# luanaruiz9/gated_gcrnns

Measured on AMD Instinct MI355X. Metric: sequences/sec (node), N=1000 K=5 T=32 F=64, higher is better.
Workload: dtype bf16

## Files before the change

### gated_gcrnns_amd/_lib.py

```python
import ctypes as C
import os

import torch

from . import build as _build

F32, F64, BF16 = 0, 1, 2

_c_i64 = C.c_int64
_c_p = C.c_void_p


class GcrnnError(RuntimeError):
    pass


def _load():
    path = os.environ.get('GCRNN_LIBPATH')
    if path:
        return _bind(C.CDLL(path))
    path = _build.LIBPATH
    if _build.needs_build() and os.path.exists(_build.HIPCC):
        _build.build(verbose=False)
    if not os.path.exists(path):
# ... 38 lines not shown
        'gcrnn_taps_backward_weight_parts': (C.c_int, [_c_i64, _c_i64, _c_i64, _c_i64, C.POINTER(_c_i64), C.POINTER(_c_i64)]),
        'gcrnn_taps_backward_weight': (C.c_int, [C.c_int, _c_p, _c_p, _c_p, _c_i64, _c_p, _c_p, C.c_double,
                                                 _c_i64, _c_i64, _c_i64, _c_i64, _c_p]),
        'gcrnn_ell_size': (C.c_int, [_c_p, _c_i64, _c_p, C.c_int, C.c_int, _c_i64, C.POINTER(_c_i64)]),
        'gcrnn_ell_fill': (C.c_int, [_c_p, _c_p, _c_p, _c_i64, _c_p, C.c_int, C.c_int, _c_i64, _c_p, _c_p, _c_p, _c_p]),
        'gcrnn_ell_assign_rows_z': (C.c_int, [_c_p, _c_p, _c_i64, _c_p, C.c_int, _c_i64, _c_i64, _c_p]),
        'gcrnn_ell_fill_z': (C.c_int, [_c_p, _c_p, _c_p, _c_i64, _c_p, C.c_int, C.c_int, _c_i64, _c_p, _c_i64, _c_p, _c_p, _c_p]),
        'gcrnn_ell_assign_rows': (C.c_int, [_c_p, _c_p, _c_i64, _c_p, C.c_int, _c_i64, _c_p]),
        'gcrnn_fused_supported': (C.c_int, [_c_i64, _c_i64, _c_i64, _c_i64]),
        'gcrnn_fused_padded_nodes': (_c_i64, []),
        'gcrnn_fused_step_waves': (_c_i64, []),
        'gcrnn_fused_wgrad_waves': (_c_i64, []),
        'gcrnn_pack_seq_major': (C.c_int, [C.c_int, _c_p, _c_p, _c_i64, _c_i64, _c_i64, _c_i64, _c_i64, _c_p, _c_p]),
        'gcrnn_pack_seq_major_padded': (C.c_int, [_c_p, _c_p] + [_c_i64] * 6 + [_c_p]),
        'gcrnn_unpack_seq_major': (C.c_int, [C.c_int, _c_p, _c_p, _c_i64, _c_i64, _c_i64, _c_i64, _c_i64, _c_p, _c_p]),
        'gcrnn_fused_pack_weights': (C.c_int, [C.c_int, _c_p, _c_p, _c_p, _c_i64, _c_i64, _c_i64, _c_i64, _c_p]),
        'gcrnn_fused_forward_bf16': (C.c_int, [_c_p, _c_p, _c_p, _c_p, _c_p, _c_p, _c_p, _c_p, _c_p, _c_p, _c_p,
                                               _c_p, _c_p,
                                               _c_i64, _c_i64, _c_i64, _c_i64, _c_i64, _c_i64, _c_i64, _c_p, C.c_int, _c_p, C.c_double, _c_p, _c_p, _c_p, _c_p]),
        'gcrnn_fused_pack_weights_wide': (C.c_int, [C.c_int, _c_p, _c_p, _c_p, _c_i64, _c_i64, _c_i64, _c_i64, _c_i64, C.c_double, _c_p]),
        'gcrnn_fused_forward_wide_supported': (C.c_int, [_c_i64] * 7 + [C.c_double, C.c_int, C.c_int]),
        'gcrnn_fused_forward_wide_bf16': (C.c_int, [_c_p] * 10 + [_c_i64] * 7 + [_c_p, C.c_int, _c_p, _c_p, _c_p, _c_p]),
        'gcrnn_fused_forward_wide_scratch_bytes': (_c_i64, [_c_i64, _c_i64, C.c_int]),
        'gcrnn_fused_forward_wide_scratch_bf16': (C.c_int, [_c_p] * 3 + [_c_i64] + [_c_p] * 7 + [_c_i64] * 7 + [_c_p, C.c_int, _c_p, _c_p, _c_p, _c_p]),
        'gcrnn_fused_backward_data_wide_supported': (C.c_int, [_c_i64] * 6 + [C.c_double, C.c_int, C.c_int]),
        'gcrnn_fused_backward_data_wide_bf16': (C.c_int, [_c_p] * 8 + [_c_i64] * 6 + [_c_p] * 7),
        'gcrnn_gate_readout_finish': (C.c_int, [_c_p, _c_i64, _c_p, _c_p, _c_p, _c_p, _c_i64, _c_p]),
        'gcrnn_fused_filter_output_wide_supported': (C.c_int, [_c_i64] * 7 + [C.c_double, C.c_int, C.c_int]),
        'gcrnn_fused_filter_output_wide_bf16': (C.c_int, [_c_p] * 7 + [_c_i64] * 7 + [_c_p, _c_p]),
        'gcrnn_fused_node_forward_wide_supported': (C.c_int, [_c_i64] * 6 + [C.c_double, C.c_int]),
        'gcrnn_fused_node_forward_wide_bf16': (C.c_int, [_c_p] * 11 + [_c_i64] * 6 + [_c_p, C.c_int, _c_p]),
        'gcrnn_fused_gate_pair_wide_supported': (C.c_int, [_c_i64] * 7 + [C.c_double, C.c_int, C.c_int]),
        'gcrnn_fused_gate_pair_prepass_wide_bf16': (C.c_int, [_c_p] * 12 + [_c_i64] * 7 + [_c_p, _c_p, _c_p, _c_p]),
        'gcrnn_fused_gate_pair_prepass_taps_wide_bf16': (C.c_int, [_c_p] * 7 + [_c_i64] + [_c_p] * 5 + [_c_i64] * 7 + [_c_p, _c_p, _c_p, _c_p]),
        'gcrnn_fused_inline_pack_supported': (C.c_int, [_c_i64, _c_i64, _c_i64, _c_i64, _c_i64, C.c_double]),
        'gcrnn_fused_seq_steps_per_launch': (_c_i64, [_c_i64] * 7 + [C.c_double, C.c_int, C.c_int, C.c_int]),
        'gcrnn_fused_filter_output_bf16': (C.c_int, [_c_p] * 11 + [_c_i64] * 7 + [C.c_double, C.c_int, _c_p]),
        'gcrnn_fused_node_forward_bf16': (C.c_int, [_c_p] * 15 + [_c_i64] * 6 + [_c_p, C.c_int, C.c_double, _c_p]),
        'gcrnn_fused_node_backward_data_bf16': (C.c_int, [_c_p] * 12 + [_c_i64] * 6 + [C.c_double, _c_p, C.c_int, _c_p]),
        'gcrnn_node_cell_backward': (C.c_int, [_c_p] * 11 + [_c_i64] * 5 + [_c_p]),
        'gcrnn_node_gate_dot': (C.c_int, [_c_p, _c_p, _c_p, _c_i64, _c_i64, _c_i64, _c_i64, _c_i64, _c_p]),
        'gcrnn_node_gate_dot_backward': (C.c_int, [_c_p, _c_p, _c_p, _c_p, _c_i64, _c_i64, _c_i64, _c_i64, _c_i64, _c_p]),
        'gcrnn_fused_edge_attention_supported': (C.c_int, [_c_i64, _c_i64]),
        'gcrnn_fused_edge_attention_bf16': (C.c_int, [_c_p] * 13 + [_c_i64] * 5 + [C.c_double, _c_p]),
        'gcrnn_fused_edge_attention_backward_supported': (C.c_int, [_c_i64, _c_i64, _c_i64]),
        'gcrnn_fused_edge_attention_backward_bf16': (C.c_int, [_c_p] * 14 + [_c_i64] * 6 + [C.c_double, _c_p]),
# ... 96 lines not shown
```

### gated_gcrnns_amd/csrc/gcrnn_fused_seq32.h

```cpp
#pragma once

#if defined(GCRNN_SEQ_STAMPS)
static __device__ unsigned long long gcrnn_seq32_stamps[256 * 96];
static __device__ __forceinline__ void gcrnn_stamp32_put(uint32_t lds_addr) {
  const unsigned long long tv = __builtin_amdgcn_s_memtime();
  asm volatile("ds_write_b64 %0, %1" ::"v"(lds_addr), "v"(tv) : "memory");
}
static __device__ __forceinline__ unsigned long long gcrnn_stamp32_get(uint32_t lds_addr) {
  unsigned long long tv;
  asm volatile("ds_read_b64 %0, %1\n\ts_waitcnt lgkmcnt(0)" : "=v"(tv) : "v"(lds_addr) : "memory");
  return tv;
}
#define GCRNN_STAMP32(slot)                                                                                   \
  do {                                                                                                        \
    if (wave == 0 && stamp_on && lane_now() == 0) gcrnn_stamp32_put((uint32_t)reinterpret_cast<uintptr_t>(smem) + M::FLAG_OFF + 8 * (slot)); \
  } while (0)
#define GCRNN_STAMP32_WAVE(slot0)                                                                             \
  do {                                                                                                        \
    if (stamp_on && lane_now() == 0) gcrnn_stamp32_put((uint32_t)reinterpret_cast<uintptr_t>(smem) + M::FLAG_OFF + 8 * ((slot0) + wave)); \
  } while (0)
#define GCRNN_STAMP32_FLUSH()                                                                                 \
  do {                                                                                                        \
    __syncthreads();                                                                                          \
    if (threadIdx.x < 96 && blockIdx.x < 256) gcrnn_seq32_stamps[blockIdx.x * 96 + threadIdx.x] = gcrnn_stamp32_get((uint32_t)reinterpret_cast<uintptr_t>(smem) + M::FLAG_OFF + 8 * threadIdx.x); \
// ... 56 lines not shown
  const int32_t* tile_nodes; const int32_t* tile_off; const uint2* ell_col4;
  int entries, B, N;
  const uint16_t* pk_src0; int64_t pksrc_stride;
  uint16_t* pk_dst0; int64_t pkdst_stride;
  int pk_stride;
  int nsteps;
  const float* gi0; const float* gf0; int64_t gstride;
  int hmod;
  const int32_t* flags;
  const float* gw;
  const uint4* tapf; float* taps_out; int ntaps;
  float* go;
  uint16_t* out1;
  const uint16_t* dh0_; int64_t dhstride;
  const uint16_t* hs0; int64_t hsstride;
  const float* gsc0; int64_t gscstride;
  float* gpart0; int64_t gpartstride;
  int final_raw;
  uint16_t* final_out; const uint16_t* final_h;
  const float* ng0; int64_t ngstride; int64_t nghalf;
  const float* r1a; const float* r1b;
  int stagger;
  uint16_t* scr;
};

__device__ __forceinline__ int lane_now() {
  int ln;
  asm volatile("v_mbcnt_lo_u32_b32 %0, -1, 0\n\tv_mbcnt_hi_u32_b32 %0, -1, %0" : "=v"(ln));
  return ln;
}

#define GCRNN_HOP_ASM_WIDE32_STREAM(D)                                                             \
  do {                                                                                             \
    const int gwbeg = tbeg[0] >> 2, gwend = tend[STILES - 1] >> 2;                                 \
    if (gwbeg < gwend) {                                                                           \
      const int ls_ = lane_now(), r = ls_ & 15, q = ls_ >> 4;                                      \
      const uint32_t colb = lds_col + r * 8 + (q >> 1) * 4;        \
      const uint32_t qh_ = (uint32_t)(q & 1) << 4;                                                 \
      asm volatile(GCRNN_HOP_ASM_WIDE32_TEXT                                                       \
                   : "+v"(D[0][0]), "+v"(D[0][1]), "+v"(D[1][0]), "+v"(D[1][1]), "+v"(D[2][0]), "+v"(D[2][1]), "+v"(D[3][0]), "+v"(D[3][1]), \
                     "+v"(D[4][0]), "+v"(D[4][1]), "+v"(D[5][0]), "+v"(D[5][1]), "+v"(D[6][0]), "+v"(D[6][1]), "+v"(D[7][0]), "+v"(D[7][1])  \
                   : "s"(GCRNN_SGPR(tend[0] >> 2)), "s"(GCRNN_SGPR(tend[1] >> 2)), "s"(GCRNN_SGPR(tend[2] >> 2)), "s"(GCRNN_SGPR(tend[3] >> 2)), \
                     "s"(GCRNN_SGPR(tend[4] >> 2)), "s"(GCRNN_SGPR(tend[5] >> 2)), "s"(GCRNN_SGPR(tend[6] >> 2)), "s"(GCRNN_SGPR(tend[7] >> 2)), \
                     "s"(GCRNN_SGPR(gwbeg)), "s"(GCRNN_SGPR(gwend - 1)), "v"(colb), "v"(qh_)               \
                   : GCRNN_HOP_ASM_WIDE32_CLOBBERS);                                               \
    }                                                                                              \
  } while (0)

template <int K, int HS, int XS>
struct Seq32Map {
  static constexpr int KS = HS + XS;
  static constexpr int PL = GCRNN_HOP_WIDE_PLANE;
  static constexpr int RS2 = 4 * NP + 16;
  static constexpr int BIAS_OFF = PL + 32 * 1024;
  static constexpr int FLAG_OFF = BIAS_OFF + 256;
  static constexpr int WOFF = 2 * PL;
  static constexpr int WB = K * KS * 2048;
  static constexpr int COL_OFF = WOFF + WB;
  static constexpr int NPCK = 128;
  static constexpr int PFS = 256;
  static_assert(16 * RS2 <= BIAS_OFF && FLAG_OFF + 768 <= WOFF, "LDS map");
  static size_t lds_bytes(int64_t entries, bool inline_pack, bool r1 = false) {
    const size_t need = (size_t)COL_OFF + (size_t)entries * 32 + GCRNN_HOP_COLUMN_PAD + NP * 4 + (r1 ? 2 * NP * 4 : 0) + (inline_pack ? (size_t)(32 * (XS > 0 ? XS : HS)) * NPCK * 2 : 0)
                        + PFS;
    return need <= 160 * 1024 ? need : 0;
  }
};

template <int K, int HS, int XS, int VAR, int MODE = 0, bool GATED = false, bool R1 = false, bool SPLIT = false>
__global__ __launch_bounds__(STHREADS) void fused_seq32_kernel(const Seq32Args a) {
  static_assert(!R1 || !SPLIT, "rank-1 graphs: every mode of the persistent form (the BPTT chain takes the adjoint plan: the factors swap)");
  static_assert(!SPLIT || ((MODE == 0 || MODE == 2) && !R1 && HS > 1), "split sequences: the (un-gated or time-gated) forward and the BPTT chain, with more than one chunk");
  constexpr bool ITEMS = (MODE == 1 || MODE == 3);
  constexpr bool SONLY = (MODE == 2 || MODE == 4);
  constexpr bool PKV = (VAR & 1) != 0, USERV = (VAR & 2) != 0 && (MODE == 0 || MODE == 4);
  constexpr bool SCRV = (VAR & 4) != 0;
  static_assert(!SCRV || (MODE == 0 && !SPLIT && (VAR & 2) != 0), "state scratch: the persistent forward with the user-layout output");
  constexpr int SCR_CH = NP * 64;
  static_assert(MODE == 0 || ((MODE >= 1 && MODE <= 4) && !GATED), "modes");
  static_assert(MODE < 3 || (!R1 && !SPLIT), "modes 3, 4: uniform-weight graphs, persistent form");
  using M = Seq32Map<K, HS, XS>;
  constexpr int KS = HS + XS;
  constexpr int F = 32 * HS, G = 32 * XS;
  constexpr int NCH = (MODE == 1) ? 2 * HS : HS;
  constexpr int PL = M::PL, WOFF = M::WOFF, WB = M::WB, COL_OFF = M::COL_OFF, RS2 = M::RS2;
  constexpr int NPCK = M::NPCK, NRND = NP / NPCK, NH = NCH * (K - 1), RPH = (NRND + NH - 1) / NH;
  constexpr int PKROWS = SONLY ? F : G;
  static_assert(STILES == 8 && GCRNN_HOP_ASM && K >= 2 && (SONLY ? XS == 0 : XS > 0), "generated hop stream: 8 tiles per wave; the chain's operand is the state alone");
  extern __shared__ __attribute__((aligned(16))) char smem[];
  const int entries = a.entries, B = a.B, N = a.N;

  const int tid = threadIdx.x, lane = tid & 63;
  const int wave = __builtin_amdgcn_readfirstlane(tid >> 6);
  const int r = lane & 15, q = lane >> 4;
  constexpr int NSPL = SPLIT ? HS : 1;
  const int wg_seq = (int)blockIdx.x / NSPL, chunk0 = SPLIT ? (int)blockIdx.x % NSPL : 0, gseq = (int)gridDim.x / NSPL;
  if (wg_seq >= B) return;

  int tbeg[STILES], tend[STILES];
#pragma unroll
// ... 41 lines not shown
          const float bv = b4[e];
          const float f = kind == 0 ? bv : (bv == 0.f ? 1.f : (kind == 1 ? __builtin_amdgcn_rcpf(bv) : bv));
          ac[h4 + e][0] *= f; ac[h4 + e][1] *= f;
        }
      }
    }
  };

  {
    const int cbytes = entries * 32;
    const char* csrc = reinterpret_cast<const char*>(a.ell_col4);
    for (int p = wave; p * 1024 < cbytes; p += SWAVES)
      if (p * 1024 + lane * 16 < cbytes)
        __builtin_amdgcn_global_load_lds((const __attribute__((address_space(1))) void*)(csrc + p * 1024 + lane * 16),
                                         (__attribute__((address_space(3))) void*)(smem + COL_OFF + p * 1024), 16, 0, 0);
    const char* wsrc = reinterpret_cast<const char*>(a.wpack) + (size_t)chunk0 * WB;
    for (int p = wave; p < WB / 1024; p += SWAVES)
      __builtin_amdgcn_global_load_lds((const __attribute__((address_space(1))) void*)(wsrc + p * 1024 + lane * 16),
                                       (__attribute__((address_space(3))) void*)(smem + WOFF + p * 1024), 16, 0, 0);
    asm volatile("s_waitcnt vmcnt(0)" ::: "memory");
  }
  if (tid < GCRNN_HOP_COLUMN_PAD / 4) reinterpret_cast<uint32_t*>(smem + COL_OFF + entries * 32)[tid] = 0u;
  float* lbias = reinterpret_cast<float*>(smem + M::BIAS_OFF);
  if (tid < NCH * 32) lbias[tid] = a.bias ? a.bias[tid] : 0.f;
  __syncthreads();

  if (a.stagger > 0) {
    const unsigned long long t0 = __builtin_amdgcn_s_memtime();
    const unsigned long long d = (unsigned long long)((blockIdx.x >> 3) & 7) * (unsigned long long)a.stagger;
    while (__builtin_amdgcn_s_memtime() - t0 < d) __builtin_amdgcn_s_sleep(16);
  }
  const uint32_t lds0 = (uint32_t)reinterpret_cast<uintptr_t>(smem);
  if (lds0 != 0) __builtin_trap();
  const uint32_t lds_col = lds0 + COL_OFF;
  char* xtile = wtab + NP * 4 + (R1 ? 2 * NP * 4 : 0);

  const int skip_hi = __builtin_amdgcn_readfirstlane((MODE == 3 || (MODE == 1 && a.flags && a.flags[0] != 0)) ? 1 : 0);
  const bool skip_h = skip_hi != 0;
  bf16x8 bfr[STILES][KS];
  auto load_first_operand = [&](int b) {
    const __amdgpu_buffer_rsrc_t rsrc_h = __builtin_amdgcn_make_buffer_rsrc(const_cast<uint16_t*>(a.hfirst), 0, skip_h ? 0 : (ITEMS ? a.hmod : B) * (NP * F * 2), 0x00020000);
    const __amdgpu_buffer_rsrc_t rsrc_x = __builtin_amdgcn_make_buffer_rsrc(const_cast<uint16_t*>(a.x0), 0, XS > 0 ? B * (NP * G * 2) : 0, 0x00020000);
    const int bh = ITEMS ? __builtin_amdgcn_readfirstlane(b % a.hmod) : b;
    const int ln0 = lane_now(), qo = ln0 >> 4;
    int sw[STILES];
    slot_words(ln0, sw);
#pragma unroll
    for (int s = 0; s < KS; ++s) {
#pragma unroll
      for (int i = 0; i < STILES; ++i) {
        const int w = sw[i];
        if (s < HS)
          bfr[i][s] = __builtin_bit_cast(bf16x8, __builtin_amdgcn_raw_buffer_load_b128(rsrc_h, (w >> 16) * (F * 2) + 16 * qo + 64 * s, bh * (NP * F * 2), 0));
        else
          bfr[i][s] = __builtin_bit_cast(bf16x8, __builtin_amdgcn_raw_buffer_load_b128(rsrc_x, (w >> 16) * (G * 2) + 16 * qo + 64 * (s - HS), b * (NP * G * 2), 0));
      }
    }
  };
  bool have_operand = false;
  for (int b = wg_seq; b < B; b += gseq) {
  if (!have_operand) load_first_operand(b);
  have_operand = false;
#pragma unroll 1
  for (int step = 0; step < a.nsteps; ++step) {
    const bool fin = (MODE == 2) && a.final_raw && step == a.nsteps - 1;
    uint16_t* hout = fin ? a.final_out : (a.out0 ? a.out0 + (int64_t)step * a.ostride : nullptr);
    [[maybe_unused]] const uint16_t* ep_dh = (SONLY && !fin && a.dh0_) ? a.dh0_ + (int64_t)step * a.dhstride : nullptr;
    [[maybe_unused]] const float* ep_ng = (MODE == 4) ? a.ng0 + (int64_t)step * a.ngstride : nullptr;
    [[maybe_unused]] const uint16_t* ep_h = (MODE == 2) ? (fin ? a.final_h : (a.hs0 ? a.hs0 + (int64_t)step * a.hsstride : nullptr)) : nullptr;
    [[maybe_unused]] float* gpart = (MODE == 2 && a.gpart0) ? a.gpart0 + (int64_t)step * a.gpartstride : nullptr;
    [[maybe_unused]] float gsc = 1.f;
    if constexpr (MODE == 2) {
      if (a.gsc0) gsc = __builtin_bit_cast(float, __builtin_amdgcn_readfirstlane(__builtin_bit_cast(int, a.gsc0[(int64_t)step * a.gscstride + b])));
    }
    float gin = 1.f, gfo = 1.f, gratio = 1.f;
    if constexpr (MODE == 4) {
      if (a.gi0) {
        gin = __builtin_bit_cast(float, __builtin_amdgcn_readfirstlane(__builtin_bit_cast(int, a.gi0[(int64_t)step * a.gstride + b])));
        gfo = __builtin_bit_cast(float, __builtin_amdgcn_readfirstlane(__builtin_bit_cast(int, a.gf0[(int64_t)step * a.gstride + b])));
      }
    }
    if constexpr (GATED) {
      gin = __builtin_bit_cast(float, __builtin_amdgcn_readfirstlane(__builtin_bit_cast(int, a.gi0[(int64_t)step * a.gstride + b])));
// ... 599 lines not shown
```

### gated_gcrnns_amd/csrc/gcrnn_fused_seq32.hip

```cpp
#include "gcrnn_fused_step.h"
#include "gcrnn_fused_seq32.h"

template <typename W>
__global__ void pack_weights_wide_kernel(const W* __restrict__ wA, const W* __restrict__ wB, uint16_t* __restrict__ out,
                                         int Fout, int F, int G, int Kin, int Kst, int K, float w) {
  const int KS = (F + G) / 32;
  const int64_t total = (int64_t)(Fout / 32) * K * 2 * KS * 64 * 8;
  const int64_t idx = (int64_t)blockIdx.x * blockDim.x + threadIdx.x;
  if (idx >= total) return;
  const int j = idx & 7, lane = (idx >> 3) & 63;
  int64_t rest = idx >> 9;
  const int s = rest % KS; rest /= KS;
  const int h = rest & 1; rest >>= 1;
  const int tap = rest % K;
  const int chunk = rest / K;
  const int m = lane & 15;
  const int f = chunk * 32 + 8 * (m >> 2) + 4 * h + (m & 3);
  const int feat = 32 * s + 8 * (lane >> 4) + j;
  float v = 0.f;
  if (feat < F) { if (tap < Kst) v = (float)wB[((int64_t)f * Kst + tap) * F + feat]; }
  else          { if (tap < Kin) v = (float)wA[((int64_t)f * Kin + tap) * G + (feat - F)]; }
  float sc = 1.f;
  for (int k = 0; k < tap; ++k) sc *= w;
  out[idx] = f2bf(v * sc);
// ... 167 lines not shown
  const size_t lds = seq32_lds<K, HS, XS>(sa.entries, inline_pack, sa.r1a != nullptr);
  if (!lds) return GCRNN_ERR_UNSUPPORTED;
  if (sa.r1a) return inline_pack ? seq32_launch_v<K, HS, XS, 1, 1, false, true>(sa, lds, st) : seq32_launch_v<K, HS, XS, 0, 1, false, true>(sa, lds, st);
  return inline_pack ? seq32_launch_v<K, HS, XS, 1, 1>(sa, lds, st) : seq32_launch_v<K, HS, XS, 0, 1>(sa, lds, st);
}

int gcrnn_seq32s_forward(const Seq32Args& sa, int K, int HS, int XS, bool inline_pack, size_t lds, hipStream_t st);

static int64_t seq32_scratch_need(int64_t B, int64_t F) {
  const int64_t wgs = B < gcrnn_persistent_grid() ? B : gcrnn_persistent_grid();
  return wgs * (F / 32 - 1) * (int64_t)NP * 64;
}

extern "C" int64_t gcrnn_fused_forward_wide_scratch_bytes(int64_t B, int64_t F, int rank1) {
  if (B <= 0 || F <= 0 || F % 32) return -1;
  const char* sw = getenv("GCRNN_SEQ32_STATE_SCRATCH");
  if (sw && sw[0] == '0') return -1;
  const char* p32 = getenv("GCRNN_SEQ32P");
  if (p32 && p32[0] != '0') return -1;
  if (!rank1 && !seq32_wanted(B) && seq32_split_wanted(B, F)) return -1;
  return seq32_scratch_need(B, F);
}

static int forward_wide_impl(const void* xs, const void* h0, void* hs, void* scratch, int64_t scratch_bytes, bool no_image, const void* wpack, const float* bias,
                             const float* gi, const float* gf, const int32_t* tile_nodes, const int32_t* tile_off, const void* ell_col4, int64_t entries,
                             int64_t B, int64_t T, int64_t N, int64_t F, int64_t G, int64_t K, void* Huser,
                             int huser_last_only, const void* Xuser_inline, const float* rank1_a, const float* rank1_b,
                             void* stream) {
  if (!xs || !h0 || (!no_image && !hs) || !wpack || !tile_nodes || !tile_off || !ell_col4) return GCRNN_ERR_NULL_POINTER;
  if (no_image && !Huser) return GCRNN_ERR_NULL_POINTER;
  if ((rank1_a == nullptr) != (rank1_b == nullptr)) return GCRNN_ERR_BAD_SHAPE;
  if ((gi == nullptr) != (gf == nullptr) || (gi && Xuser_inline)) return GCRNN_ERR_BAD_SHAPE;
  if (B <= 0 || T <= 0 || N <= 0 || N > NP || B > (1 << 24) || entries <= 0 || entries % 4) return GCRNN_ERR_BAD_SHAPE;
  if (B * (NP * (F > G ? F : G) * 2) > 2147483647LL || T * F * N > 2147483647LL) return GCRNN_ERR_BAD_SHAPE;
  if (Huser && (N % 8 != 0 || (reinterpret_cast<uintptr_t>(Huser) & 15))) return GCRNN_ERR_BAD_SHAPE;
  if (Xuser_inline && (N % 8 != 0 || (reinterpret_cast<uintptr_t>(Xuser_inline) & 15) || T * G * N > 2147483647LL)) return GCRNN_ERR_BAD_SHAPE;
  if (no_image) {
    if (F % 32 || F < 32) return GCRNN_ERR_UNSUPPORTED;
    const int64_t need = seq32_scratch_need(B, F);
    if (scratch_bytes < need || (need > 0 && (!scratch || (reinterpret_cast<uintptr_t>(scratch) & 15)))) return GCRNN_ERR_BAD_SHAPE;
  }
  const int64_t xstep = B * NP * G, hstep = B * NP * F;
  Seq32Args sa{};
  sa.x0 = (const uint16_t*)xs; sa.xstride = xstep;
  sa.hfirst = (const uint16_t*)h0;
  sa.out0 = no_image ? nullptr : (uint16_t*)hs; sa.ostride = hstep;
  sa.scr = no_image ? (uint16_t*)scratch : nullptr;
  sa.wpack = (const uint4*)wpack; sa.bias = bias;
  sa.a1 = (const uint16_t*)Huser; sa.a1stride = F * N; sa.a1_last_only = huser_last_only ? 1 : 0;
  sa.ubstride = (int)((huser_last_only ? 1 : T) * F * N);
  sa.tile_nodes = tile_nodes; sa.tile_off = tile_off; sa.ell_col4 = (const uint2*)ell_col4;
  sa.entries = (int)entries; sa.B = (int)B; sa.N = (int)N;
  sa.nsteps = (int)T;
  sa.gi0 = gi; sa.gf0 = gf; sa.gstride = B;
  sa.r1a = rank1_a; sa.r1b = rank1_b;
  {
    const char* sg = getenv("GCRNN_SEQ32_STAGGER");
    sa.stagger = sg ? atoi(sg) : 0;
  }
  const bool inline_pack = Xuser_inline != nullptr && T > 2;
  if (inline_pack) {
    sa.pk_src0 = (const uint16_t*)Xuser_inline; sa.pksrc_stride = G * N;
    sa.pk_dst0 = const_cast<uint16_t*>(sa.x0); sa.pkdst_stride = xstep;
    sa.pk_stride = (int)(T * G * N);
  }
  hipStream_t st = as_stream(stream);
  const bool split = !rank1_a && !seq32_wanted(B) && seq32_split_wanted(B, F);
  if (no_image) {
    if (split) return GCRNN_ERR_UNSUPPORTED;
#define GCRNN_SEQ32_CASE(KK, HH, XX) \
    if (K == KK && F == 32 * HH && G == 32 * XX) { \
      const size_t lds = seq32_lds<KK, HH, XX>(sa.entries, inline_pack, sa.r1a != nullptr); \
      return lds ? gcrnn_seq32s_forward(sa, KK, HH, XX, inline_pack, lds, st) : GCRNN_ERR_UNSUPPORTED; \
    }
    GCRNN_SEQ32_CASE(5, 2, 2) GCRNN_SEQ32_CASE(4, 2, 2) GCRNN_SEQ32_CASE(3, 2, 2) GCRNN_SEQ32_CASE(2, 2, 2)
    GCRNN_SEQ32_CASE(5, 2, 1) GCRNN_SEQ32_CASE(4, 2, 1) GCRNN_SEQ32_CASE(3, 2, 1) GCRNN_SEQ32_CASE(2, 2, 1)
    GCRNN_SEQ32_CASE(5, 1, 1) GCRNN_SEQ32_CASE(4, 1, 1) GCRNN_SEQ32_CASE(3, 1, 1) GCRNN_SEQ32_CASE(2, 1, 1)
#undef GCRNN_SEQ32_CASE
    return GCRNN_ERR_UNSUPPORTED;
  }
  const bool pack_split = Xuser_inline != nullptr && T > 1;
  if (split && pack_split && !inline_pack) {
    sa.pk_src0 = (const uint16_t*)Xuser_inline; sa.pksrc_stride = G * N;
    sa.pk_dst0 = const_cast<uint16_t*>(sa.x0); sa.pkdst_stride = xstep;
    sa.pk_stride = (int)(T * G * N);
  }
#define GCRNN_SEQ32_CASE(KK, HH, XX) if (K == KK && F == 32 * HH && G == 32 * XX) return seq32_launch<KK, HH, XX>(sa, split ? pack_split : inline_pack, st, split, T, N);
  GCRNN_SEQ32_CASE(5, 2, 2) GCRNN_SEQ32_CASE(4, 2, 2) GCRNN_SEQ32_CASE(3, 2, 2) GCRNN_SEQ32_CASE(2, 2, 2)
  GCRNN_SEQ32_CASE(5, 2, 1) GCRNN_SEQ32_CASE(4, 2, 1) GCRNN_SEQ32_CASE(3, 2, 1) GCRNN_SEQ32_CASE(2, 2, 1)
  GCRNN_SEQ32_CASE(5, 1, 1) GCRNN_SEQ32_CASE(4, 1, 1) GCRNN_SEQ32_CASE(3, 1, 1) GCRNN_SEQ32_CASE(2, 1, 1)
#undef GCRNN_SEQ32_CASE
  return GCRNN_ERR_UNSUPPORTED;
}

extern "C" int gcrnn_fused_forward_wide_bf16(const void* xs, const void* h0, void* hs, const void* wpack, const float* bias,
                                             const float* gi, const float* gf, const int32_t* tile_nodes, const int32_t* tile_off, const void* ell_col4, int64_t entries,
                                             int64_t B, int64_t T, int64_t N, int64_t F, int64_t G, int64_t K, void* Huser,
                                             int huser_last_only, const void* Xuser_inline, const float* rank1_a, const float* rank1_b,
                                             void* stream) {
  return forward_wide_impl(xs, h0, hs, nullptr, 0, false, wpack, bias, gi, gf, tile_nodes, tile_off, ell_col4, entries, B, T, N, F, G, K, Huser,
                           huser_last_only, Xuser_inline, rank1_a, rank1_b, stream);
}

extern "C" int gcrnn_fused_forward_wide_scratch_bf16(const void* xs, const void* h0, void* scratch, int64_t scratch_bytes, const void* wpack, const float* bias,
                                                     const float* gi, const float* gf, const int32_t* tile_nodes, const int32_t* tile_off, const void* ell_col4,
                                                     int64_t entries, int64_t B, int64_t T, int64_t N, int64_t F, int64_t G, int64_t K, void* Huser,
                                                     int huser_last_only, const void* Xuser_inline, const float* rank1_a, const float* rank1_b,
                                                     void* stream) {
  return forward_wide_impl(xs, h0, nullptr, scratch, scratch_bytes, true, wpack, bias, gi, gf, tile_nodes, tile_off, ell_col4, entries, B, T, N, F, G, K, Huser,
                           huser_last_only, Xuser_inline, rank1_a, rank1_b, stream);
}


extern "C" int gcrnn_fused_gate_pair_wide_supported(int64_t B, int64_t T, int64_t N, int64_t F, int64_t G, int64_t K, int64_t entries,
                                                    double uniform_w, int img16, int with_pack) {
  if (uniform_w == 0.0 || !img16 || N <= 0 || N > NP || B <= 0 || T <= 0 || entries <= 0 || entries % 4) return 0;
  if (with_pack && (N % 8 || T * G * N > 2147483647LL)) return 0;
  if (B * T * (NP * (F > G ? F : G) * 2) > 2147483647LL) return 0;
  if (!seq32_wanted(B * T)) return 0;
  if (!seq32_lds_for(F, G, K, entries, with_pack != 0, (img16 & 2) != 0)) return 0;
  if (!with_pack) return 1;
  const int64_t first = B * T < gcrnn_persistent_grid() ? B * T : gcrnn_persistent_grid();
  return (int)((first + B - 1) / B);
}

static int gate_pair_prepass_impl(const void* x_user, void* xs, const void* h0, const void* wpack, const float* bias2,
                                  const float* gw2, float* parts, const void* tapf, float* taps_out, int64_t ntaps, void* cs_in, void* cs_f,
                                  const int32_t* tile_nodes, const int32_t* tile_off, const void* ell_col4, int64_t entries, int64_t B, int64_t T,
                                  int64_t N, int64_t F, int64_t G, int64_t K, const int32_t* h0_zero_flag,
                                  const float* rank1_a, const float* rank1_b, void* stream) {
  if (!xs || !h0 || !wpack || !tile_nodes || !tile_off || !ell_col4) return GCRNN_ERR_NULL_POINTER;
  if (tapf ? (!taps_out || ntaps <= 0 || ntaps > 16 || (reinterpret_cast<uintptr_t>(tapf) & 15)) : (!gw2 || !parts)) return GCRNN_ERR_NULL_POINTER;
  if ((rank1_a == nullptr) != (rank1_b == nullptr)) return GCRNN_ERR_NULL_POINTER;
// ... 169 lines not shown
```

### gated_gcrnns_amd/ops.py

```python
import ctypes as C
import os

import torch

from . import _lib
from ._lib import lib, check, dtype_code, GcrnnError


def _p(t):
    return C.c_void_p(t.data_ptr()) if t is not None else None


def _stream():
    return C.c_void_p(torch.cuda.current_stream().cuda_stream)


def require_device(*tensors):
    for t in tensors:
        if t is not None and not t.is_cuda:
            raise GcrnnError('gated_gcrnns_amd has no CPU path: move the module and its inputs to a ROCm '
                             'device (model.to("cuda"), x.cuda()); got a tensor on %s' % t.device)


def _pack_raw(x, perm=None):
# ... 289 lines not shown
    wpack = torch.empty(((F // 16) * K * ((F + G) // 32) * 64 * 8,), dtype=torch.bfloat16, device=dev)
    wAc, wBc = wA.contiguous(), wB.contiguous()
    check(lib.gcrnn_fused_pack_weights(dtype_code(wA.dtype), _p(wAc), _p(wBc), _p(wpack),
                                       F, G, Kin, Kst, st), 'pack_weights')
    b32 = bias.detach().float().contiguous().view(-1) if bias is not None else None
    H = torch.empty((B, T, F, N), dtype=torch.bfloat16, device=dev) if (N % 8 == 0 and user_layout) else None
    e0, e1 = torch.cuda.Event(enable_timing=True), torch.cuda.Event(enable_timing=True)
    ok = fused_inline_pack_ok(plan, N, F, G, K)
    inline_arg = inline
    inline = (ok if inline is None else (ok and inline)) and X.data_ptr() % 16 == 0
    plan16 = fused_img16_plan(graph, False, None)
    wide = fused_wide_plan(graph, B, T, N, F, G, K, inline)
    if wide is None and plan16 is None:
        inl1 = inline_arg is not False and not os.environ.get('GCRNN_NO_INLINE_PACK') and X.data_ptr() % 16 == 0
        wide = fused_wide_plan(graph, B, T, N, F, G, K, inl1, rank1=True)
        if wide is None and inl1:
            inl1 = False
            wide = fused_wide_plan(graph, B, T, N, F, G, K, False, rank1=True)
        if wide is not None:
            inline = inl1
    if wide is not None:
        wpw = _fused_pack_weights_wide(wAc, wBc, wide['uniform_w'], st)
        scr = fused_state_scratch(wide, B, F, dev) if H is not None else None
        for rep in range(reps + warm):
            if rep == warm:
                e0.record()
            _fused_forward_wide(wide, xs, h0s, hs, wAc, wBc, b32, B, T, N, F, G, K, H, False, Xc if inline else None, st, wpw=wpw, scratch=scr)
        e1.record()
        torch.cuda.synchronize()
        per_step = 1e3 * e0.elapsed_time(e1) / (reps * T)
        return {'avg_us': per_step, 'launches': reps, 'inline_pack': bool(inline), 'steps_per_launch': T,
                'launch_avg_us': per_step * T, 'kernel': 'fused_seq32_kernel'}
    for rep in range(reps + 1):
        if rep == 1:
            torch.cuda.synchronize()
            e0.record()
        check(lib.gcrnn_fused_forward_bf16(_p(xs), _p(h0s), _p(hs), _p(wpack), _p(b32), None, None, *_fused_graph_args(plan16 or plan),
                                           B, T, N, F, G, K, _p(H) if H is not None else None, 2 if plan16 else 0, None, plan.get('uniform_w', 0.0),
                                           _p(Xc) if inline else None, None, None, st),
              'fused_forward')
    e1.record()
    torch.cuda.synchronize()
    spl = int(lib.gcrnn_fused_seq_steps_per_launch(B, T, N, F, G, K, int((plan16 or plan)['entries']), float(plan.get('uniform_w', 0.0)),
                                                   1 if plan16 else 0, 1 if inline else 0, 0))
    per_step = 1e3 * e0.elapsed_time(e1) / (reps * T)
    return {'avg_us': per_step, 'launches': reps * T // max(spl, 1), 'inline_pack': bool(inline), 'steps_per_launch': max(spl, 1),
            'launch_avg_us': per_step * max(spl, 1), 'kernel': 'fused_seq_kernel' if spl else 'fused_step_kernel'}


# ... 68 lines not shown
    Kin, Kst = wA.shape[2], wB.shape[2]
    K = max(Kin, Kst)

    def make():
        wpack = torch.empty(((Fout // 32) * K * 2 * ((F + G) // 32) * 64 * 8,), dtype=torch.bfloat16, device=wA.device)
        wAc, wBc, kin = wA.contiguous(), wB.contiguous(), Kin
        if G == 0:
            wAc, kin = wBc, Kst
        check(lib.gcrnn_fused_pack_weights_wide(dtype_code(wB.dtype), _p(wAc), _p(wBc), _p(wpack), Fout, F, G, kin, Kst, float(uniform_w), st),
              'pack_weights_wide')
        return wpack
    return _cached_pack('taps32', (wA.detach(), wB.detach()), float(uniform_w), st, make)


def fused_wide_plan(graph, B, T, N, F, G, K, inline, rank1=False, gated=False):
    plan16 = fused_img16_plan(graph, False, None)
    if plan16 is None and rank1 and not os.environ.get('GCRNN_NO_IMG16'):
        plan16 = graph.fused_plan_rank1()
    if plan16 is None or F % 32 or G % 32:
        return None
    ok = lib.gcrnn_fused_forward_wide_supported(int(B), int(T), int(N), int(F), int(G), int(K), int(plan16['entries']),
                                                float(plan16.get('uniform_w', 0.0)), (3 if plan16.get('rank1') else 1) | (4 if gated else 0), 1 if inline else 0)
    return plan16 if ok else None


def fused_state_scratch(plan16, B, F, dev):
    need = int(lib.gcrnn_fused_forward_wide_scratch_bytes(int(B), int(F), 1 if plan16.get('rank1') else 0))
    if need < 0:
        return None
    return torch.empty((need,), dtype=torch.uint8, device=dev)


def _fused_forward_wide(plan16, xs, h0s, hs, wA, wB, b32, B, T, N, F, G, K, H, last_only, Xinline, st, wpw=None, gi=None, gf=None, scratch=None):
    if wpw is None:
        wpw = _fused_pack_weights_wide(wA.detach(), wB.detach(), plan16['uniform_w'], st)
    if scratch is not None:
        assert H is not None
        check(lib.gcrnn_fused_forward_wide_scratch_bf16(_p(xs), _p(h0s), _p(scratch), int(scratch.numel()), _p(wpw), _p(b32), _p(gi), _p(gf), _p(plan16['tile_slots']),
                                                        _p(plan16['tile_off']), _p(plan16['ell_col4']), plan16['entries'], B, T, N, F, G, K,
                                                        _p(H), int(bool(last_only)), _p(Xinline) if Xinline is not None else None,
                                                        _p(plan16.get('rank1_a')), _p(plan16.get('rank1_b')), st),
              'fused_forward_wide_scratch')
        return
    check(lib.gcrnn_fused_forward_wide_bf16(_p(xs), _p(h0s), _p(hs), _p(wpw), _p(b32), _p(gi), _p(gf), _p(plan16['tile_slots']), _p(plan16['tile_off']),
                                            _p(plan16['ell_col4']), plan16['entries'], B, T, N, F, G, K,
                                            _p(H) if H is not None else None, int(bool(last_only)), _p(Xinline) if Xinline is not None else None,
# ... 212 lines not shown
                       last_only=False, head=None, native_out=False):
    require_device(X, h0, wA, wB, bias)
    if packed is None and X.shape[2] < wA.shape[3]:
        if X.shape[3] % 2 == 0 and X.dtype == torch.bfloat16:
            packed = fused_pack_inputs(X, h0, graph, channels=wA.shape[3])
        else:
            Xz = X.new_zeros((X.shape[0], X.shape[1], wA.shape[3], X.shape[3]))
            Xz[:, :, :X.shape[2]] = X
            X = Xz
    elif packed is None:
        X, wA = fused_pad_operands(X, wA.detach())
    B, T, _, N = X.shape
    G = wA.shape[3]
    F = wA.shape[0]
    K = max(wA.shape[2], wB.shape[2])
    plan = graph.fused_plan()
    st = _stream()
    dev = X.device
    X = X.contiguous()
    h0 = h0.contiguous()
    events = None
    inline = False
    lean = packed is None and head is None and not return_states and not native_out and N % 8 == 0
    if packed is not None:
        xs, hs_all = packed
    elif gates is None and gate_values is None and X.data_ptr() % 16 == 0 and (
            fused_inline_pack_ok(plan, N, F, G, K) or (head is None and not os.environ.get('GCRNN_NO_INLINE_PACK')
                                                       and fused_wide_plan(graph, B, T, N, F, G, K, True, rank1=True) is not None)):
        xs, hs_all = fused_pack_inputs(X, h0, graph, first_only=True, states=not lean)
        inline = True
    elif gates is None and fused_overlap_ok(X):
        xs, hs_all, events = fused_pack_inputs(X, h0, graph, overlap=True, states=not lean)
    elif gates is not None and gate_values is None:
        xs, hs_all = fused_pack_inputs_gated(X, h0, graph, F, K, states=not lean)
    else:
        xs, hs_all = fused_pack_inputs(X, h0, graph, states=not lean)
    h0s, hs = hs_all[:1], hs_all[1:]
    gi = gf = None
    if gate_values is not None:
        gi, gf = (g.detach().float().contiguous() for g in gate_values)
        assert tuple(gi.shape) == (T, B) and tuple(gf.shape) == (T, B)
    elif gates is not None:
        hzero = fused_h0_zero_flag(h0)
        g = {}
        gp = {}
        for name in ('in', 'forget'):
# ... 2214 lines not shown
```

### include/gcrnn.h

```cpp
#ifndef GCRNN_H
#define GCRNN_H

#include <stdint.h>

#ifdef __cplusplus
extern "C" {
#endif

enum { GCRNN_F32 = 0, GCRNN_F64 = 1, GCRNN_BF16 = 2 };

enum {
  GCRNN_OK = 0,
  GCRNN_ERR_BAD_DTYPE = 1,
  GCRNN_ERR_BAD_SHAPE = 2,
  GCRNN_ERR_NULL_POINTER = 3,
  GCRNN_ERR_UNSUPPORTED = 4,
  GCRNN_ERR_LAUNCH = 5,
  GCRNN_ERR_WORKSPACE = 6
};

int gcrnn_version(void);
const char* gcrnn_status_string(int status);
const char* gcrnn_last_hip_error(void);

// ... 160 lines not shown
                             int64_t entries, int64_t B, int64_t T, int64_t N, int64_t F, int64_t G, int64_t K,
                             void* Huser, int huser_last_only, void* const* step_events, double uniform_w,
                             const void* Xuser_inline ,
                             const float* head_w ,
                             float* head_part ,
                             void* stream);

int gcrnn_fused_pack_weights_wide(int wdtype, const void* wA, const void* wB, void* wpack, int64_t Fout, int64_t F, int64_t G, int64_t Kin,
                                  int64_t Kst, double uniform_w, void* stream);
int gcrnn_fused_forward_wide_supported(int64_t B, int64_t T, int64_t N, int64_t F, int64_t G, int64_t K, int64_t entries, double uniform_w,
                                       int img16, int inline_pack);
int gcrnn_fused_forward_wide_bf16(const void* xs, const void* h0, void* hs, const void* wpack, const float* bias, const float* gi,
                                  const float* gf, const int32_t* tile_nodes, const int32_t* tile_off, const void* ell_col4, int64_t entries,
                                  int64_t B, int64_t T, int64_t N, int64_t F, int64_t G, int64_t K, void* Huser, int huser_last_only,
                                  const void* Xuser_inline,
                                  const float* rank1_a, const float* rank1_b ,
                                  void* stream);
int64_t gcrnn_fused_forward_wide_scratch_bytes(int64_t B, int64_t F, int rank1);
int gcrnn_fused_forward_wide_scratch_bf16(const void* xs, const void* h0, void* scratch, int64_t scratch_bytes, const void* wpack,
                                          const float* bias, const float* gi, const float* gf, const int32_t* tile_nodes,
                                          const int32_t* tile_off, const void* ell_col4, int64_t entries, int64_t B, int64_t T, int64_t N,
                                          int64_t F, int64_t G, int64_t K, void* Huser, int huser_last_only, const void* Xuser_inline,
                                          const float* rank1_a, const float* rank1_b, void* stream);
int gcrnn_fused_gate_pair_wide_supported(int64_t B, int64_t T, int64_t N, int64_t F, int64_t G, int64_t K, int64_t entries, double uniform_w,
                                         int img16, int with_pack);
int gcrnn_fused_backward_data_wide_supported(int64_t B, int64_t T, int64_t N, int64_t F, int64_t K, int64_t entries, double uniform_w, int img16,
                                             int inline_pack);
int gcrnn_fused_backward_data_wide_bf16(const void* dHs, const void* hs, void* dpre, void* dh0, const void* wpackT, const int32_t* tile_nodes,
                                        const int32_t* tile_off, const void* ell_col4, int64_t entries, int64_t B, int64_t T, int64_t N,
                                        int64_t F, int64_t K, const float* gf, const void* h0s, float* dgf_parts, const void* dHuser_inline,
                                        const float* rank1_a, const float* rank1_b, void* stream);
int gcrnn_fused_filter_output_wide_supported(int64_t B, int64_t T, int64_t N, int64_t F, int64_t G, int64_t K, int64_t entries, double uniform_w,
                                             int img16, int with_pack );
int gcrnn_fused_filter_output_wide_bf16(const void* xs, const void* wpack, const float* bias, void* out, const int32_t* tile_nodes,
                                        const int32_t* tile_off, const void* ell_col4, int64_t entries, int64_t B, int64_t T, int64_t N,
                                        int64_t F, int64_t G, int64_t K,
                                        const void* x_user ,
                                        void* stream);
int gcrnn_fused_node_forward_wide_supported(int64_t B, int64_t T, int64_t N, int64_t F, int64_t K, int64_t entries, double uniform_w, int img16);
int gcrnn_fused_node_forward_wide_bf16(const void* h0s, void* hs, const void* yx, const float* ngates, const float* gi, const float* gf,
                                       const void* wpackB, const float* bias, const int32_t* tile_nodes, const int32_t* tile_off,
                                       const void* ell_col4, int64_t entries, int64_t B, int64_t T, int64_t N, int64_t F, int64_t K, void* Huser,
                                       int huser_last_only, void* stream);
int gcrnn_gate_readout_finish(const float* parts, int64_t nparts, const float* lb_in, const float* lb_f, float* gi, float* gf, int64_t items,
                              void* stream);
int gcrnn_fused_gate_pair_prepass_wide_bf16(const void* x_user, void* xs, const void* h0, const void* wpack, const float* bias2,
// ... 165 lines not shown
```

Baseline: 161,800.

## Fold h0 and first input layout packing into persistent forward kernel prologue

Adds a prologue inside the persistent seq32 forward kernel that transposes the user-layout h0 and the first one or two input steps into the padded sequence-major layout. It uses LDS-staged DMA loads, swizzled reads and buffer stores. It also lets the kernel read a bf16 bias directly. This removes the separate pack and conversion launches before the forward pass on the lean path. In exchange it adds prologue work inside each per-sequence loop and passes state through a thread-local handoff set by a new API call.

```diff
diff --git a/gated_gcrnns_amd/_lib.py b/gated_gcrnns_amd/_lib.py
--- a/gated_gcrnns_amd/_lib.py
+++ b/gated_gcrnns_amd/_lib.py
@@ -84,6 +84,8 @@
         'gcrnn_fused_forward_wide_supported': (C.c_int, [_c_i64] * 7 + [C.c_double, C.c_int, C.c_int]),
         'gcrnn_fused_forward_wide_bf16': (C.c_int, [_c_p] * 10 + [_c_i64] * 7 + [_c_p, C.c_int, _c_p, _c_p, _c_p, _c_p]),
         'gcrnn_fused_forward_wide_scratch_bytes': (_c_i64, [_c_i64, _c_i64, C.c_int]),
+        'gcrnn_fused_forward_wide_user_supported': (C.c_int, [_c_i64] * 7 + [C.c_double, C.c_int]),
+        'gcrnn_fused_forward_wide_user_next': (C.c_int, [_c_p, C.c_int]),
         'gcrnn_fused_forward_wide_scratch_bf16': (C.c_int, [_c_p] * 3 + [_c_i64] + [_c_p] * 7 + [_c_i64] * 7 + [_c_p, C.c_int, _c_p, _c_p, _c_p, _c_p]),
         'gcrnn_fused_backward_data_wide_supported': (C.c_int, [_c_i64] * 6 + [C.c_double, C.c_int, C.c_int]),
         'gcrnn_fused_backward_data_wide_bf16': (C.c_int, [_c_p] * 8 + [_c_i64] * 6 + [_c_p] * 7),
diff --git a/gated_gcrnns_amd/csrc/gcrnn_fused_seq32.h b/gated_gcrnns_amd/csrc/gcrnn_fused_seq32.h
--- a/gated_gcrnns_amd/csrc/gcrnn_fused_seq32.h
+++ b/gated_gcrnns_amd/csrc/gcrnn_fused_seq32.h
@@ -102,6 +102,8 @@
   const float* r1a; const float* r1b;
   int stagger;
   uint16_t* scr;
+  const uint16_t* pro_h0;
+  int bias_bf16;
 };
 
 __device__ __forceinline__ int lane_now() {
@@ -126,6 +128,18 @@
                    : GCRNN_HOP_ASM_WIDE32_CLOBBERS);                                               \
     }                                                                                              \
   } while (0)
+
+__device__ __forceinline__ void seq32_tile_read16(uint32_t a0, uint32_t a1, uint32_t (&h0)[8], uint32_t (&h1)[8]) {
+  asm volatile("ds_read_u16 %0, %16\n\tds_read_u16 %1, %16 offset:256\n\tds_read_u16 %2, %16 offset:512\n\tds_read_u16 %3, %16 offset:768\n\t"
+               "ds_read_u16 %4, %16 offset:1024\n\tds_read_u16 %5, %16 offset:1280\n\tds_read_u16 %6, %16 offset:1536\n\tds_read_u16 %7, %16 offset:1792\n\t"
+               "ds_read_u16 %8, %17\n\tds_read_u16 %9, %17 offset:256\n\tds_read_u16 %10, %17 offset:512\n\tds_read_u16 %11, %17 offset:768\n\t"
+               "ds_read_u16 %12, %17 offset:1024\n\tds_read_u16 %13, %17 offset:1280\n\tds_read_u16 %14, %17 offset:1536\n\tds_read_u16 %15, %17 offset:1792\n\t"
+               "s_waitcnt lgkmcnt(0)"
+               : "=&v"(h0[0]), "=&v"(h0[1]), "=&v"(h0[2]), "=&v"(h0[3]), "=&v"(h0[4]), "=&v"(h0[5]), "=&v"(h0[6]), "=&v"(h0[7]),
+                 "=&v"(h1[0]), "=&v"(h1[1]), "=&v"(h1[2]), "=&v"(h1[3]), "=&v"(h1[4]), "=&v"(h1[5]), "=&v"(h1[6]), "=&v"(h1[7])
+               : "v"(a0), "v"(a1)
+               : "memory");
+}
 
 template <int K, int HS, int XS>
 struct Seq32Map {
@@ -156,6 +170,7 @@
   constexpr bool PKV = (VAR & 1) != 0, USERV = (VAR & 2) != 0 && (MODE == 0 || MODE == 4);
   constexpr bool SCRV = (VAR & 4) != 0;
   static_assert(!SCRV || (MODE == 0 && !SPLIT && (VAR & 2) != 0), "state scratch: the persistent forward with the user-layout output");
+  constexpr bool PROV = PKV && SCRV && !GATED;
   constexpr int SCR_CH = NP * 64;
   static_assert(MODE == 0 || ((MODE >= 1 && MODE <= 4) && !GATED), "modes");
   static_assert(MODE < 3 || (!R1 && !SPLIT), "modes 3, 4: uniform-weight graphs, persistent form");
@@ -243,7 +258,7 @@
   }
   if (tid < GCRNN_HOP_COLUMN_PAD / 4) reinterpret_cast<uint32_t*>(smem + COL_OFF + entries * 32)[tid] = 0u;
   float* lbias = reinterpret_cast<float*>(smem + M::BIAS_OFF);
-  if (tid < NCH * 32) lbias[tid] = a.bias ? a.bias[tid] : 0.f;
+  if (tid < NCH * 32) lbias[tid] = !a.bias ? 0.f : (a.bias_bf16 ? bf2f(reinterpret_cast<const uint16_t*>(a.bias)[tid]) : a.bias[tid]);
   __syncthreads();
 
   if (a.stagger > 0) {
@@ -278,8 +293,85 @@
       }
     }
   };
+  [[maybe_unused]] auto pro_layout = [&](auto rowsc, const uint16_t* src, uint16_t* dst, int b, int nr) __attribute__((always_inline)) {
+    constexpr int ROWS = decltype(rowsc)::value;
+    constexpr int TB = ROWS * NPCK * 2, NB = 65536 / TB;
+    constexpr int PPR = NPCK / 8, PPT = ROWS * PPR / STHREADS;
+    constexpr int PCS = ROWS / 8, NPC = NB * PCS * NPCK / STHREADS;
+    static_assert(ROWS * PPR % STHREADS == 0 && NB * TB <= M::BIAS_OFF && NPC % 2 == 0 && (STHREADS % PCS) == 0, "prologue tiles");
+    static_assert(NPCK * 2 == 256, "row pitch of the pack tile in seq32_tile_read16");
+    typedef __attribute__((__vector_size__(4 * sizeof(unsigned int)))) unsigned int u32x4_t;
+    const __amdgpu_buffer_rsrc_t rsrc_d = __builtin_amdgcn_make_buffer_rsrc(dst, 0, B * (NP * ROWS * 2), 0x00020000);
+#pragma unroll 1
+    for (int r0 = 0; r0 < nr; r0 += NB) {
+      const int tl = wave * 64 + lane_now();
+#pragma unroll
+      for (int k = 0; k < NB; ++k) {
+        if (r0 + k < nr) {
+#pragma unroll
+          for (int i = 0; i < PPT; ++i) {
+            const int id = i * STHREADS + tl;
+            const int row = id / PPR, cs = id - row * PPR;
+            const int col = (cs - (row >> 3)) & (PPR - 1);
+            if ((r0 + k) * NPCK + col * 8 < N)
+              __builtin_amdgcn_global_load_lds((const __attribute__((address_space(1))) void*)(src + (int64_t)row * N + (r0 + k) * NPCK + col * 8),
+                                               (__attribute__((address_space(3))) void*)(smem + k * TB + (i * STHREADS + wave * 64) * 16), 16, 0, GCRNN_SEQ32_NT_DMA);
+          }
+        }
+      }
+      asm volatile("s_waitcnt vmcnt(0)" ::: "memory");
+      lds_barrier();
+      u32x4_t vv[NPC];
+#pragma unroll
+      for (int j = 0; j < NPC; j += 2) {
+        uint32_t h16[2][8], sa[2];
+#pragma unroll
+        for (int e = 0; e < 2; ++e) {
+          const int k = (j + e) / (NPC / NB), id = ((j + e) % (NPC / NB)) * STHREADS + tl;
+          const int nl = id / PCS, pc = id - nl * PCS;
+          sa[e] = (uint32_t)(k * TB + (pc * 8) * (NPCK * 2) + ((nl + 8 * pc) & (NPCK - 1)) * 2);
+        }
+        seq32_tile_read16(sa[0], sa[1], h16[0], h16[1]);
+#pragma unroll
+        for (int e = 0; e < 2; ++e) {
+          const int k = (j + e) / (NPC / NB), id = ((j + e) % (NPC / NB)) * STHREADS + tl;
+          const bool ok = (r0 + k) * NPCK + id / PCS < N;
+          uint32_t w4[4];
+#pragma unroll
+          for (int jj = 0; jj < 4; ++jj) w4[jj] = h16[e][2 * jj] | (h16[e][2 * jj + 1] << 16);
+          vv[j + e] = u32x4_t{ok ? w4[0] : 0u, ok ? w4[1] : 0u, ok ? w4[2] : 0u, ok ? w4[3] : 0u};
+        }
+      }
+      int so[NPC];
+#pragma unroll
+      for (int j = 0; j < NPC; ++j) {
+        const int k = j / (NPC / NB), id = (j % (NPC / NB)) * STHREADS + tl;
+        const int nl = id / PCS, pc = id - nl * PCS;
+        so[j] = ((r0 + k) * NPCK + nl) * (ROWS * 2) + pc * 16 + b * (NP * ROWS * 2);
+      }
+#pragma unroll
+      for (int j = 0; j < NPC; ++j) asm volatile("" : "+v"(vv[j]), "+v"(so[j]));
+#pragma unroll
+      for (int j = 0; j < NPC; ++j) {
+        const int k = j / (NPC / NB);
+        if (r0 + k < nr) __builtin_amdgcn_raw_buffer_store_b128(vv[j], rsrc_d, so[j], 0, 0);
+      }
+      asm volatile("s_nop 3" ::: "memory");
+      lds_barrier();
+    }
+  };
   bool have_operand = false;
   for (int b = wg_seq; b < B; b += gseq) {
+  if constexpr (PROV) {
+    if (a.pro_h0) {
+      pro_layout(std::integral_constant<int, F>{}, a.pro_h0 + (int64_t)b * (F * N), const_cast<uint16_t*>(a.hfirst), b, NRND);
+      pro_layout(std::integral_constant<int, G>{}, a.pk_src0 + (int64_t)b * a.pk_stride, const_cast<uint16_t*>(a.x0), b, NRND);
+      if (a.nsteps > 1)
+        pro_layout(std::integral_constant<int, G>{}, a.pk_src0 + (int64_t)b * a.pk_stride + a.pksrc_stride, const_cast<uint16_t*>(a.x0) + a.xstride, b, NRND);
+      asm volatile("s_waitcnt vmcnt(0)" ::: "memory");
+      lds_barrier();
+    }
+  }
   if (!have_operand) load_first_operand(b);
   have_operand = false;
 #pragma unroll 1
diff --git a/gated_gcrnns_amd/csrc/gcrnn_fused_seq32.hip b/gated_gcrnns_amd/csrc/gcrnn_fused_seq32.hip
--- a/gated_gcrnns_amd/csrc/gcrnn_fused_seq32.hip
+++ b/gated_gcrnns_amd/csrc/gcrnn_fused_seq32.hip
@@ -213,13 +213,22 @@
   return seq32_scratch_need(B, F);
 }
 
+extern "C" int gcrnn_fused_forward_wide_user_supported(int64_t B, int64_t T, int64_t N, int64_t F, int64_t G, int64_t K, int64_t entries,
+                                                       double uniform_w, int img16) {
+  const char* sw = getenv("GCRNN_SEQ32_PROLOGUE");
+  if (sw && sw[0] == '0') return 0;
+  if (gcrnn_fused_forward_wide_scratch_bytes(B, F, (img16 & 2) != 0) < 0) return 0;
+  return gcrnn_fused_forward_wide_supported(B, T, N, F, G, K, entries, uniform_w, img16, 1);
+}
+
 static int forward_wide_impl(const void* xs, const void* h0, void* hs, void* scratch, int64_t scratch_bytes, bool no_image, const void* wpack, const float* bias,
                              const float* gi, const float* gf, const int32_t* tile_nodes, const int32_t* tile_off, const void* ell_col4, int64_t entries,
                              int64_t B, int64_t T, int64_t N, int64_t F, int64_t G, int64_t K, void* Huser,
                              int huser_last_only, const void* Xuser_inline, const float* rank1_a, const float* rank1_b,
-                             void* stream) {
+                             void* stream, const void* h0_user = nullptr, bool bias_bf16 = false) {
   if (!xs || !h0 || (!no_image && !hs) || !wpack || !tile_nodes || !tile_off || !ell_col4) return GCRNN_ERR_NULL_POINTER;
   if (no_image && !Huser) return GCRNN_ERR_NULL_POINTER;
+  if (h0_user && (!no_image || !Xuser_inline || gi || (reinterpret_cast<uintptr_t>(h0_user) & 15))) return GCRNN_ERR_BAD_SHAPE;
   if ((rank1_a == nullptr) != (rank1_b == nullptr)) return GCRNN_ERR_BAD_SHAPE;
   if ((gi == nullptr) != (gf == nullptr) || (gi && Xuser_inline)) return GCRNN_ERR_BAD_SHAPE;
   if (B <= 0 || T <= 0 || N <= 0 || N > NP || B > (1 << 24) || entries <= 0 || entries % 4) return GCRNN_ERR_BAD_SHAPE;
@@ -237,7 +246,8 @@
   sa.hfirst = (const uint16_t*)h0;
   sa.out0 = no_image ? nullptr : (uint16_t*)hs; sa.ostride = hstep;
   sa.scr = no_image ? (uint16_t*)scratch : nullptr;
-  sa.wpack = (const uint4*)wpack; sa.bias = bias;
+  sa.wpack = (const uint4*)wpack; sa.bias = bias; sa.bias_bf16 = bias_bf16 ? 1 : 0;
+  sa.pro_h0 = (const uint16_t*)h0_user;
   sa.a1 = (const uint16_t*)Huser; sa.a1stride = F * N; sa.a1_last_only = huser_last_only ? 1 : 0;
   sa.ubstride = (int)((huser_last_only ? 1 : T) * F * N);
   sa.tile_nodes = tile_nodes; sa.tile_off = tile_off; sa.ell_col4 = (const uint2*)ell_col4;
@@ -249,7 +259,7 @@
     const char* sg = getenv("GCRNN_SEQ32_STAGGER");
     sa.stagger = sg ? atoi(sg) : 0;
   }
-  const bool inline_pack = Xuser_inline != nullptr && T > 2;
+  const bool inline_pack = Xuser_inline != nullptr && (T > 2 || h0_user);
   if (inline_pack) {
     sa.pk_src0 = (const uint16_t*)Xuser_inline; sa.pksrc_stride = G * N;
     sa.pk_dst0 = const_cast<uint16_t*>(sa.x0); sa.pkdst_stride = xstep;
@@ -293,13 +303,29 @@
                            huser_last_only, Xuser_inline, rank1_a, rank1_b, stream);
 }
 
+static thread_local const void* seq32_next_h0_user = nullptr;
+static thread_local int seq32_next_bias_dtype = GCRNN_F32;
+
+extern "C" int gcrnn_fused_forward_wide_user_next(const void* h0_user, int bias_dtype) {
+  if (!h0_user) return GCRNN_ERR_NULL_POINTER;
+  if (bias_dtype != GCRNN_F32 && bias_dtype != GCRNN_BF16) return GCRNN_ERR_BAD_DTYPE;
+  if (reinterpret_cast<uintptr_t>(h0_user) & 15) return GCRNN_ERR_BAD_SHAPE;
+  seq32_next_h0_user = h0_user;
+  seq32_next_bias_dtype = bias_dtype;
+  return GCRNN_OK;
+}
+
 extern "C" int gcrnn_fused_forward_wide_scratch_bf16(const void* xs, const void* h0, void* scratch, int64_t scratch_bytes, const void* wpack, const float* bias,
                                                      const float* gi, const float* gf, const int32_t* tile_nodes, const int32_t* tile_off, const void* ell_col4,
                                                      int64_t entries, int64_t B, int64_t T, int64_t N, int64_t F, int64_t G, int64_t K, void* Huser,
                                                      int huser_last_only, const void* Xuser_inline, const float* rank1_a, const float* rank1_b,
                                                      void* stream) {
+  const void* h0_user = seq32_next_h0_user;
+  const bool bias_bf16 = h0_user && seq32_next_bias_dtype == GCRNN_BF16;
+  seq32_next_h0_user = nullptr;
+  if (h0_user && B > 0 && N > 0 && F > 0 && B * F * N > 2147483647LL) return GCRNN_ERR_BAD_SHAPE;
   return forward_wide_impl(xs, h0, nullptr, scratch, scratch_bytes, true, wpack, bias, gi, gf, tile_nodes, tile_off, ell_col4, entries, B, T, N, F, G, K, Huser,
-                           huser_last_only, Xuser_inline, rank1_a, rank1_b, stream);
+                           huser_last_only, Xuser_inline, rank1_a, rank1_b, stream, h0_user, bias_bf16);
 }
 
 
diff --git a/gated_gcrnns_amd/ops.py b/gated_gcrnns_amd/ops.py
--- a/gated_gcrnns_amd/ops.py
+++ b/gated_gcrnns_amd/ops.py
@@ -335,9 +335,15 @@
     if wide is not None:
         wpw = _fused_pack_weights_wide(wAc, wBc, wide['uniform_w'], st)
         scr = fused_state_scratch(wide, B, F, dev) if H is not None else None
+        user = None
+        if scr is not None and inline and inline_arg is not False and h0c.data_ptr() % 16 == 0 and X.dtype == torch.bfloat16 and h0.dtype == torch.bfloat16:
+            user = fused_wide_user_plan(graph, B, T, N, F, G, K, bias)
         for rep in range(reps + warm):
             if rep == warm:
                 e0.record()
+            if user is not None:
+                _fused_forward_wide_user(user, Xc, h0c, xs, h0s, scr, wAc, wBc, bias, B, T, N, F, G, K, H, False, st, wpw=wpw)
+                continue
             _fused_forward_wide(wide, xs, h0s, hs, wAc, wBc, b32, B, T, N, F, G, K, H, False, Xc if inline else None, st, wpw=wpw, scratch=scr)
         e1.record()
         torch.cuda.synchronize()
@@ -452,6 +458,28 @@
     ok = lib.gcrnn_fused_forward_wide_supported(int(B), int(T), int(N), int(F), int(G), int(K), int(plan16['entries']),
                                                 float(plan16.get('uniform_w', 0.0)), (3 if plan16.get('rank1') else 1) | (4 if gated else 0), 1 if inline else 0)
     return plan16 if ok else None
+
+
+def fused_wide_user_plan(graph, B, T, N, F, G, K, bias=None):
+    if bias is not None and (bias.dtype not in (torch.float32, torch.bfloat16) or not bias.is_contiguous()):
+        return None
+    plan16 = fused_wide_plan(graph, B, T, N, F, G, K, True, rank1=True)
+    if plan16 is None:
+        return None
+    ok = lib.gcrnn_fused_forward_wide_user_supported(int(B), int(T), int(N), int(F), int(G), int(K), int(plan16['entries']),
+                                                     float(plan16.get('uniform_w', 0.0)), 3 if plan16.get('rank1') else 1)
+    return plan16 if ok else None
+
+
+def _fused_forward_wide_user(plan16, X, h0, xs, h0s, scratch, wA, wB, bias, B, T, N, F, G, K, H, last_only, st, wpw=None):
+    if wpw is None:
+        wpw = _fused_pack_weights_wide(wA.detach(), wB.detach(), plan16['uniform_w'], st)
+    bd = bias.detach() if bias is not None else None
+    check(lib.gcrnn_fused_forward_wide_user_next(_p(h0), dtype_code(bd.dtype) if bd is not None else _lib.F32), 'fused_forward_wide_user_next')
+    check(lib.gcrnn_fused_forward_wide_scratch_bf16(_p(xs), _p(h0s), _p(scratch), int(scratch.numel()), _p(wpw), _p(bd), None, None, _p(plan16['tile_slots']),
+                                                    _p(plan16['tile_off']), _p(plan16['ell_col4']), plan16['entries'], B, T, N, F, G, K,
+                                                    _p(H), int(bool(last_only)), _p(X), _p(plan16.get('rank1_a')), _p(plan16.get('rank1_b')), st),
+          'fused_forward_wide_scratch')
 
 
 def fused_state_scratch(plan16, B, F, dev):
@@ -710,6 +738,17 @@
     events = None
     inline = False
     lean = packed is None and head is None and not return_states and not native_out and N % 8 == 0
+    wide_user = None
+    if lean and gates is None and gate_values is None and X.data_ptr() % 16 == 0 and h0.data_ptr() % 16 == 0 and X.dtype == torch.bfloat16 \
+            and h0.dtype == torch.bfloat16 and not os.environ.get('GCRNN_NO_INLINE_PACK'):
+        wide_user = fused_wide_user_plan(graph, B, T, N, F, G, K, bias)
+    if wide_user is not None:
+        xs = torch.empty((T, B, plan['npad'], G), dtype=torch.bfloat16, device=dev)
+        hs_all = torch.empty((1, B, plan['npad'], F), dtype=torch.bfloat16, device=dev)
+        scr = fused_state_scratch(wide_user, B, F, dev)
+        H = torch.empty((B, 1 if last_only else T, F, N), dtype=torch.bfloat16, device=dev)
+        _fused_forward_wide_user(wide_user, X, h0, xs, hs_all, scr, wA, wB, bias, B, T, N, F, G, K, H, last_only, st)
+        return H
     if packed is not None:
         xs, hs_all = packed
     elif gates is None and gate_values is None and X.data_ptr() % 16 == 0 and (
diff --git a/include/gcrnn.h b/include/gcrnn.h
--- a/include/gcrnn.h
+++ b/include/gcrnn.h
@@ -206,6 +206,9 @@
                                           const int32_t* tile_off, const void* ell_col4, int64_t entries, int64_t B, int64_t T, int64_t N,
                                           int64_t F, int64_t G, int64_t K, void* Huser, int huser_last_only, const void* Xuser_inline,
                                           const float* rank1_a, const float* rank1_b, void* stream);
+int gcrnn_fused_forward_wide_user_supported(int64_t B, int64_t T, int64_t N, int64_t F, int64_t G, int64_t K, int64_t entries,
+                                            double uniform_w, int img16);
+int gcrnn_fused_forward_wide_user_next(const void* h0_user, int bias_dtype);
 int gcrnn_fused_gate_pair_wide_supported(int64_t B, int64_t T, int64_t N, int64_t F, int64_t G, int64_t K, int64_t entries, double uniform_w,
                                          int img16, int with_pack);
 int gcrnn_fused_backward_data_wide_supported(int64_t B, int64_t T, int64_t N, int64_t F, int64_t K, int64_t entries, double uniform_w, int img16,
```

Result: no change. 162,500 (median of 6 runs) (+0.5%).
